# tokamak-network/Tokamak-zk-EVM

Measured on AMD Instinct MI355X. Metric: constraints/sec (prove step), higher is better.
Workload: dtype u32 limbs (255-bit Fr / 381-bit Fq modular integer arithmetic)

## Files before the change

tokamak-zk-evm_amd/csrc/msm.hip:

```cpp
#include <stdio.h>
#include <stdlib.h>

#include <algorithm>
#include <map>
#include <memory>
#include <mutex>
#include <thread>
#include <vector>

#include "common.h"
#include "ec_u.h"

#define TK_MSM_PRIMARY 1
#define TK_MSM_NS tk_msm_bls12_381
#define TK_MSM_FR_PARAMS bls12_381_fr_params
#define TK_MSM_FQ_PARAMS bls12_381_fq_params
#define TK_MSM_SCALAR_BITS 255
#define TK_MSM_ABI_FR tkmk_fr
#define TK_MSM_ABI_AFFINE tkmk_g1_affine
#define TK_MSM_ABI_PROJ tkmk_g1_projective
#define TK_MSM_ABI_JOB tkmk_msm_job
#define TK_MSM_SYM_MSM bls12_381_msm
#define TK_MSM_SYM_MULTI tkmk_msm_multi
#define TK_MSM_SYM_PRECOMPUTE bls12_381_msm_precompute_bases
#define TK_MSM_SYM_PRECOMPUTE_ACC bls12_381_msm_precompute_bases_acc
#define TK_MSM_ABI_JOB_EX tkmk_msm_job_ex
#define TK_MSM_SYM_MULTI_EX tkmk_msm_multi_ex
#define TK_MSM_SYM_CONVERT bls12_381_msm_convert_bases
#define TK_MSM_SYM_SEGMENTED tkmk_msm_segmented
#define TK_MSM_SYM_SEGMENTED_STATUS tkmk_msm_segmented_status
#include "msm_impl.inc"
```

tokamak-zk-evm_amd/csrc/msm_bn254.hip:

```cpp
#include <stdio.h>
#include <stdlib.h>

#include <algorithm>
#include <map>
#include <memory>
#include <mutex>
#include <vector>

#include "common.h"
#include "ec_u.h"

#define TK_MSM_NS tk_msm_bn254
#define TK_MSM_FR_PARAMS bn254_fr_params
#define TK_MSM_FQ_PARAMS bn254_fq_params
#define TK_MSM_SCALAR_BITS 254
#define TK_MSM_ABI_FR tkmk_bn254_fr
#define TK_MSM_ABI_AFFINE tkmk_bn254_g1_affine
#define TK_MSM_ABI_PROJ tkmk_bn254_g1_projective
#define TK_MSM_ABI_JOB tkmk_bn254_msm_job
#define TK_MSM_SYM_MSM bn254_msm
#define TK_MSM_SYM_MULTI tkmk_bn254_msm_multi
#define TK_MSM_SYM_PRECOMPUTE bn254_msm_precompute_bases
#include "msm_impl.inc"
```

tokamak-zk-evm_amd/csrc/msm_impl.inc:

```
namespace TK_MSM_NS {

using FrP = TK_MSM_FR_PARAMS;
using FqP = TK_MSM_FQ_PARAMS;
using Fr = ff<FrP>;
using Fq = ff<FqP>;
using fr_t = Fr::E;
using fq_t = Fq::E;
using G1 = ec<Fq>;
using g1_affine_t = affine_t<Fq>;
using g1_xyzz_t = xyzz_t<Fq>;
using G1U = ecu<FqP>;
using G1K = G1;
using FqK = Fq;
using g1k_xyzz = g1_xyzz_t;
using g1k_aff = g1_affine_t;
using abi_fr = TK_MSM_ABI_FR;
using abi_affine = TK_MSM_ABI_AFFINE;
using abi_proj = TK_MSM_ABI_PROJ;
using abi_job = TK_MSM_ABI_JOB;
#ifdef TK_MSM_SYM_MULTI_EX
using abi_job_ex = TK_MSM_ABI_JOB_EX;
#endif
constexpr size_t AFF_BYTES = sizeof(g1_affine_t), FR_BYTES = sizeof(fr_t);
#ifdef TK_MSM_SYM_PRECOMPUTE_ACC
// ... 46 lines not shown
__device__ __forceinline__ uint32_t view_at_expanded(const msm_view_t &v, uint32_t k, uint32_t n_src, uint32_t level_rows) {
    if (!level_rows) return view_at(v, k);
    uint32_t j = k / n_src;
    return j * level_rows + view_at(v, k - j * n_src);
}
static inline msm_view_t view_identity() { return msm_view_t{nullptr, 0, 0, 0, nullptr}; }
static inline bool view_is_identity(const msm_view_t &v) { return !v.index && !v.cols; }

__global__ __launch_bounds__(256) void k_convert_bases(const g1_affine_t *__restrict__ in, g1_affine_t *__restrict__ out,
                                                      uint64_t n, int in_montgomery, msm_view_t bv) {
    uint64_t i = (uint64_t)blockIdx.x * blockDim.x + threadIdx.x;
    if (i >= n) return;
    g1_affine_t p = tk_load(in + view_at(bv, (uint32_t)i));
    if (!G1::is_inf(p)) {
        fq_t k;
#pragma unroll
        for (int j = 0; j < Fq::N; j++) k.l[j] = in_montgomery ? FqP::KSATM[j] : FqP::KSAT[j];
        p.x = Fq::mul(Fq::canon(p.x), k);
        p.y = Fq::mul(Fq::canon(p.y), k);
    }
    tk_store(out + i, p);
}

__global__ __launch_bounds__(256) void k_digits(const fr_t *__restrict__ scalars, uint32_t *__restrict__ dig, msm_plan_t pl,
                                               int scalars_mont, msm_view_t sv) {
    uint32_t i = blockIdx.x * blockDim.x + threadIdx.x;
    if (i >= pl.n_src) return;
    fr_t s = Fr::canon(tk_load(scalars + view_at(sv, i)));
    if (scalars_mont) s = Fr::from_mont(s);
    uint32_t carry = 0;
    const uint32_t mask = (1u << pl.c) - 1u;
    const uint32_t groups = pl.n / pl.n_src;
    uint32_t j = 0, t = 0;
    for (uint32_t w = 0; w < groups * pl.W; w++) {
        if (w >= pl.W_src) {
            dig[(uint64_t)t * pl.n + (uint64_t)j * pl.n_src + i] = 0;
            if (++t == pl.W) { t = 0; j++; }
            continue;
        }
        uint32_t lo = w * pl.c, li = lo >> 5, sh = lo & 31;
        uint32_t raw = 0;
        if (li < 8) {
            raw = s.l[li] >> sh;
            if (sh + pl.c > 32 && li + 1 < 8) raw |= s.l[li + 1] << (32 - sh);
        }
        raw &= mask;
        if (lo + pl.c > pl.bits) {
            uint32_t keep = pl.bits > lo ? pl.bits - lo : 0;
            raw &= keep >= 32 ? 0xffffffffu : ((1u << keep) - 1u);
        }
        uint32_t v = raw + carry;
        uint32_t rec;
        if (v > pl.B) {
            rec = ((1u << pl.c) - v) | 0x80000000u;
            carry = 1;
        } else {
            rec = v;
            carry = 0;
        }
        dig[(uint64_t)t * pl.n + (uint64_t)j * pl.n_src + i] = rec;
        if (++t == pl.W) { t = 0; j++; }
    }
}

template <class Out>
__device__ __forceinline__ void precompute_bases_body(const g1_affine_t *__restrict__ in, Out *__restrict__ out, uint64_t n, int in_montgomery,
                                                      uint32_t factor, uint32_t step) {
    uint64_t i = (uint64_t)blockIdx.x * blockDim.x + threadIdx.x;
    if (i >= n) return;
    g1_affine_t p = tk_load(in + i);
    const bool inf = G1::is_inf(p);
    if (!inf) {
        p.x = Fq::canon(p.x);
        p.y = Fq::canon(p.y);
        if (!in_montgomery) {
            p.x = Fq::to_mont(p.x);
            p.y = Fq::to_mont(p.y);
        }
    }
    fq_t k;
#pragma unroll
    for (int l = 0; l < Fq::N; l++) k.l[l] = FqP::KSATM[l];
    g1_xyzz_t acc = G1::from_affine(p);
    for (uint32_t j = 0; j < factor; j++) {
        g1_affine_t a = p;
// ... 25 lines not shown
                                              uint32_t shift) {
    extern __shared__ uint32_t hist[];
    const uint32_t w = blockIdx.y, ch = blockIdx.x;
    for (uint32_t b = threadIdx.x; b < pl.B; b += blockDim.x) hist[b] = 0;
    __syncthreads();
    uint32_t lo = ch * pl.chunk_len, hi = lo + pl.chunk_len;
    if (hi > pl.n) hi = pl.n;
    const uint32_t *d = dig + (uint64_t)w * pl.n;
    uint32_t i = lo + threadIdx.x;
    for (; i + 3 * 1024 < hi; i += 4 * 1024) {
        uint32_t r[4];
#pragma unroll
        for (int j = 0; j < 4; j++) r[j] = d[i + 1024 * j] & 0x7fffffffu;
#pragma unroll
        for (int j = 0; j < 4; j++)
            if (r[j]) atomicAdd(&hist[(r[j] - 1) >> shift], 1u);
    }
    for (; i < hi; i += 1024) {
        uint32_t r = d[i] & 0x7fffffffu;
        if (r) atomicAdd(&hist[(r - 1) >> shift], 1u);
    }
    __syncthreads();
    uint32_t *c = counts + (uint64_t)w * pl.B * pl.chunks;
    for (uint32_t b = threadIdx.x; b < pl.B; b += blockDim.x) c[(uint64_t)b * pl.chunks + ch] = hist[b];
}

__global__ __launch_bounds__(1024) void k_scan_local(const uint32_t *__restrict__ counts, uint32_t *__restrict__ local,
                                                    uint32_t *__restrict__ gtot, msm_plan_t pl) {
    __shared__ uint32_t part[1024];
    const uint32_t w = blockIdx.y, t = threadIdx.x, b = blockIdx.x * 1024 + t;
    uint32_t sum = 0;
    if (b < pl.B) {
        const uint32_t *c = counts + ((uint64_t)w * pl.B + b) * pl.chunks;
        uint32_t k = 0;
        for (; k + 8 <= pl.chunks; k += 8) {
            uint32_t v[8];
#pragma unroll
            for (int j = 0; j < 8; j++) v[j] = c[k + j];
#pragma unroll
            for (int j = 0; j < 8; j++) sum += v[j];
        }
        for (; k < pl.chunks; k++) sum += c[k];
    }
    part[t] = sum;
    __syncthreads();
    for (uint32_t off = 1; off < 1024; off <<= 1) {
// ... 114 lines not shown
    uint32_t *s = sorted + (uint64_t)w * pl.n;
    for (uint32_t i = lo + threadIdx.x; i < hi; i += blockDim.x) {
        uint32_t rec = d[i];
        uint32_t r = rec & 0x7fffffffu;
        if (r) {
            uint32_t pos = atomicAdd(&cur[r - 1], 1u);
            s[pos] = view_at_expanded(bv, i, pl.n_src, level_rows) | (rec & 0x80000000u);
        }
    }
}

#ifndef SC_TILE
#define SC_TILE 4096
#endif
#define SC_PER (SC_TILE / 1024)
#define SC_MAXBINS 1024
#define SC_MAXFINE 512
#define SC_PARTS 4
__device__ __forceinline__ uint32_t sc_part_len(uint32_t len, uint32_t parts) {
    uint32_t per = (len + parts - 1) / parts;
    return (per + SC_TILE - 1) / SC_TILE * SC_TILE;
}

template <bool PASS_B>
__global__ __launch_bounds__(1024) void k_scatter_staged(const uint32_t *__restrict__ in0, const uint16_t *__restrict__ in1,
                                                        const uint32_t *__restrict__ seg_start, const uint32_t *__restrict__ cursors,
                                                        uint32_t *__restrict__ out0, uint16_t *__restrict__ out1, uint32_t n,
                                                        uint32_t bins, uint32_t coarse_bins, uint32_t chunk_len, uint32_t fbits,
                                                        msm_view_t bv, uint32_t n_src, uint32_t level_rows) {
    __shared__ uint32_t hist[SC_MAXBINS], start[SC_MAXBINS], cur[SC_MAXBINS], wsum[16];
    const uint32_t fmask = (1u << fbits) - 1;
    __shared__ uint32_t sv0[SC_TILE], sv1[SC_TILE];
    const uint32_t tid = threadIdx.x, parts = gridDim.x, sgm = blockIdx.y;
    uint32_t part = blockIdx.x;
    if ((parts & 7u) == 0) part = (blockIdx.x & 7u) * (parts >> 3) + (blockIdx.x >> 3);
    const uint32_t w = PASS_B ? sgm / coarse_bins : sgm;
    uint32_t lo, hi, base = 0;
    if (PASS_B) {
        const uint32_t cb = sgm - w * coarse_bins;
        const uint32_t *cs = seg_start + (uint64_t)w * (coarse_bins + 1);
        uint32_t s0 = cs[cb], s1 = cs[cb + 1];
        uint32_t per = sc_part_len(s1 - s0, parts);
        lo = s0 + part * per;
        if (lo > s1) lo = s1;
        hi = lo + per < s1 ? lo + per : s1;
        base = s0;
    } else {
        lo = part * chunk_len;
        hi = lo + chunk_len < n ? lo + chunk_len : n;
        if (lo > n) lo = n;
    }
    in0 += (uint64_t)w * n;
    if (PASS_B) in1 += (uint64_t)w * n;
    out0 += (uint64_t)w * n;
    if (!PASS_B) out1 += (uint64_t)w * n;
    if (tid < bins) cur[tid] = cursors[((uint64_t)sgm * bins + tid) * parts + part] + base;
    hist[tid] = 0;
    __syncthreads();
    for (uint32_t tlo = lo; tlo < hi; tlo += SC_TILE) {
        uint32_t v0[SC_PER], v1[SC_PER], rk[SC_PER];
        bool ok[SC_PER];
#pragma unroll
        for (int j = 0; j < SC_PER; j++) {
            uint32_t k = tlo + tid + 1024u * j;
            ok[j] = k < hi;
            v0[j] = v1[j] = rk[j] = 0;
            if (ok[j]) {
                if (PASS_B) {
                    v0[j] = in0[k];
                    v1[j] = in1[k];
                } else {
                    uint32_t rec = in0[k], r = rec & 0x7fffffffu;
                    ok[j] = r != 0;
                    v0[j] = (ok[j] ? view_at_expanded(bv, k, n_src, level_rows) : 0u) | (rec & 0x80000000u);
                    v1[j] = r - 1;
                }
            }
            if (ok[j]) rk[j] = atomicAdd(&hist[PASS_B ? (v1[j] & fmask) : (v1[j] >> fbits)], 1u);
        }
        __syncthreads();
        static_assert(SC_MAXBINS == 1024, "one bin per thread of the 1024-thread workgroup");
        const uint32_t mine = hist[tid];
        uint32_t incl = mine;
        const uint32_t lane = tid & 63u, wave = tid >> 6;
#pragma unroll
        for (uint32_t off = 1; off < 64; off <<= 1) {
            uint32_t t = __shfl_up(incl, off, 64);
            if (lane >= off) incl += t;
        }
        if (lane == 63) wsum[wave] = incl;
        __syncthreads();
        uint32_t before = 0, total = 0;
#pragma unroll
        for (uint32_t w2 = 0; w2 < 16; w2++) {
            uint32_t v = wsum[w2];
            total += v;
            if (w2 < wave) before += v;
        }
        start[tid] = before + incl - mine;
        __syncthreads();
#pragma unroll
        for (int j = 0; j < SC_PER; j++)
            if (ok[j]) {
                uint32_t b = PASS_B ? (v1[j] & fmask) : (v1[j] >> fbits);
                uint32_t pos = start[b] + rk[j];
                sv0[pos] = v0[j];
                sv1[pos] = v1[j];
            }
        __syncthreads();
#pragma unroll
        for (int j = 0; j < SC_PER; j++) {
            uint32_t k2 = tid + 1024u * j;
            if (k2 < total) {
                uint32_t a0 = sv0[k2], a1 = sv1[k2];
                uint32_t b = PASS_B ? (a1 & fmask) : (a1 >> fbits);
                uint32_t g = cur[b] + (k2 - start[b]);
                out0[g] = a0;
                if (!PASS_B) out1[g] = (uint16_t)(a1 & fmask);
            }
        }
        __syncthreads();
        cur[tid] += hist[tid];
        hist[tid] = 0;
        __syncthreads();
    }
}

__global__ __launch_bounds__(1024) void k_hist_fine(const uint16_t *__restrict__ key, const uint32_t *__restrict__ seg_start,
                                                   uint32_t *__restrict__ counts, uint32_t n, uint32_t coarse_bins, uint32_t fbits) {
    __shared__ uint32_t hist[SC_MAXFINE];
    const uint32_t fb_n = 1u << fbits;
    const uint32_t tid = threadIdx.x, part = blockIdx.x, parts = gridDim.x, sgm = blockIdx.y;
    const uint32_t w = sgm / coarse_bins, cb = sgm - w * coarse_bins;
    const uint32_t *cs = seg_start + (uint64_t)w * (coarse_bins + 1);
    uint32_t s0 = cs[cb], s1 = cs[cb + 1];
    uint32_t per = sc_part_len(s1 - s0, parts);
    uint32_t lo = s0 + part * per;
    if (lo > s1) lo = s1;
    uint32_t hi = lo + per < s1 ? lo + per : s1;
    if (tid < fb_n) hist[tid] = 0;
    __syncthreads();
    const uint16_t *k = key + (uint64_t)w * n;
    uint32_t i = lo + tid;
    for (; i + 3 * 1024 < hi; i += 4 * 1024) {
        uint32_t r[4];
#pragma unroll
        for (int j = 0; j < 4; j++) r[j] = k[i + 1024 * j];
// ... 656 lines not shown
    if (getenv("TKMK_MSM_FIXED_CHUNK")) return MSM_CHUNK;
    if (const char *e = getenv("TKMK_MSM_CHUNK_LEN")) {
        int v = atoi(e);
        if (v >= 8 && v <= 8192) return (uint32_t)v;
    }
    uint64_t target = entries / (8ull * slots);
    if (target < 48) target = 48;
    if (target > 224) target = 224;
    uint64_t r = (entries + target * slots / 2) / (target * slots);
    if (r < 1) r = 1;
    uint64_t lanes_per_window = r * slots / W;
    if (lanes_per_window < 1) lanes_per_window = 1;
    uint64_t chunk = (n + lanes_per_window - 1) / lanes_per_window;
    if (chunk < 32) chunk = 32;
    if (chunk > 256) chunk = 256;
    if (entries > (1ull << 30)) {
        uint64_t big = entries / (32ull * slots);
        if (big > 4096) big = 4096;
        if (big > chunk) chunk = big;
    }
    return (uint32_t)chunk;
}
#define MSM_MAX_C 20
static uint32_t msm_resolve_c(uint32_t c_req, uint32_t n_src) {
    uint32_t c = c_req ? c_req : choose_c(n_src);
    if (c < 2) c = 2;
    if (c > MSM_MAX_C) c = MSM_MAX_C;
    static const bool force_one_pass = getenv("TKMK_MSM_ONE_PASS") != nullptr;
    if (c > 16 && (force_one_pass || n_src < (1u << 18))) c = 16;
    return c;
}

struct msm_acc_lds_t {
    uint32_t foreground, background;
};
static const msm_acc_lds_t &msm_acc_lds() {
    static const msm_acc_lds_t claims = [] {
        const char *fg = getenv("TKMK_MSM_ACC_LDS"), *bg = getenv("TKMK_MSM_BACKGROUND_LDS");
        msm_acc_lds_t v{fg ? (uint32_t)atoi(fg) : 0u, bg ? (uint32_t)atoi(bg) : 98304u};
        const int most = (int)(v.foreground > v.background ? v.foreground : v.background);
        hipError_t e = most ? hipFuncSetAttribute((const void *)k_accumulate_chunks, hipFuncAttributeMaxDynamicSharedMemorySize, most) : hipSuccess;
#ifdef TK_MSM_SYM_PRECOMPUTE_ACC
        if (most && e == hipSuccess) e = hipFuncSetAttribute((const void *)k_accumulate_chunks_rows, hipFuncAttributeMaxDynamicSharedMemorySize, most);
#endif
        if (e != hipSuccess) v = msm_acc_lds_t{0, 0};
        return v;
    }();
    return claims;
}
static tkmk_error msm_enqueue(const fr_t *scalars, const g1_affine_t *bases_mont, uint32_t n_src, uint32_t factor, uint32_t c_req,
                              uint32_t bits, bool scalars_mont, hipStream_t s, g1_xyzz_t *wins_host, msm_plan_t *plan_out, bool background,
                              msm_view_t sv = view_identity(), msm_view_t bv = view_identity(), uint32_t level_rows = 0,
// ... 16 lines not shown
    pl.B = 1u << (pl.c - 1);
    pl.chunk = msm_choose_chunk((uint64_t)pl.W * n, pl.W, n);
    {
        static const uint32_t big_env = getenv("TKMK_MSM_BIG") ? (uint32_t)atoi(getenv("TKMK_MSM_BIG")) : 0u;
        const uint64_t avg_spans = (uint64_t)n / ((uint64_t)pl.chunk * pl.B);
        pl.big = big_env ? big_env : (avg_spans >= 4 ? 4u * MSM_BIG : MSM_BIG);
    }
    pl.win_parts = pl.W >= 8 ? MSM_WIN_PARTS : 32;
    pl.hi_bits = pl.lo_bits = 0;
    if (pl.W == 1 && pl.c >= 15) {
        pl.lo_bits = (pl.c - 1) / 2;
        pl.hi_bits = pl.c - 1 - pl.lo_bits;
    }
    static const bool no_rowcol = getenv("TKMK_MSM_SEGMENT_TAIL") != nullptr;
    if (no_rowcol) pl.hi_bits = pl.lo_bits = 0;
    uint32_t want = (512 + pl.W - 1) / pl.W;
    if (getenv("TKMK_MSM_CHUNKS")) want = (uint32_t)atoi(getenv("TKMK_MSM_CHUNKS"));
    uint32_t maxc = (n + 8191) / 8192;
    pl.chunks = want < maxc ? want : maxc;
    if (pl.chunks < 1) pl.chunks = 1;
    pl.chunk_len = (n + pl.chunks - 1) / pl.chunks;

    tk_scratch d_dig, d_sorted, d_counts, d_bstart, d_buckets, d_segs, d_wins;
    TK_TRY(d_dig.alloc((size_t)pl.W * n * 4, s));
    TK_TRY(d_sorted.alloc((size_t)pl.W * n * 4, s));
    const bool two_pass = !force_one_pass && pl.c >= 13 && n >= (1u << 18);
    if (pl.c > 16 && !two_pass) return TKMK_ERR_INVALID_ARGUMENT;
    {
        const uint32_t fb = pl.c >= 19 ? 9u : pl.c >= 17 ? 8u : 7u;
        TK_TRY(d_counts.alloc((size_t)pl.W * (two_pass ? (pl.B >> fb) : pl.B) * pl.chunks * 4, s));
    }
    TK_TRY(d_bstart.alloc((size_t)pl.W * (pl.B + 1) * 4, s));
    TK_TRY(d_buckets.alloc((size_t)pl.W * pl.B * sizeof(g1_xyzz_t), s));
    uint32_t segs = (pl.B + MSM_SEG - 1) / MSM_SEG;
    TK_TRY(d_segs.alloc((size_t)pl.W * segs * sizeof(g1_xyzz_t), s));
    TK_TRY(d_wins.alloc((size_t)pl.W * pl.win_parts * sizeof(g1_xyzz_t), s));

    tk_stat_add(TK_STAT_MSM_POINTS, n_src);
    tk_stat_add(TK_STAT_MSM_CALLS, 1);
    tk_prof prof(s);
    hipLaunchKernelGGL(k_digits, tk_div_up(n_src, 256), 256, 0, s, scalars, d_dig.as<uint32_t>(), pl, scalars_mont ? 1 : 0, sv);
    prof.mark("msm.digits");
    size_t lds = (size_t)pl.B * 4;
    static std::once_flag attr_once;
    static hipError_t attr_err = hipSuccess;
    std::call_once(attr_once, [] {
        attr_err = hipFuncSetAttribute((const void *)k_hist, hipFuncAttributeMaxDynamicSharedMemorySize, 128 * 1024);
        if (attr_err == hipSuccess)
            attr_err = hipFuncSetAttribute((const void *)k_scatter, hipFuncAttributeMaxDynamicSharedMemorySize, 128 * 1024);
    });
    TK_HIP(attr_err);
    if (!two_pass) {
        hipLaunchKernelGGL(k_hist, dim3(pl.chunks, pl.W), 1024, lds, s, (const uint32_t *)d_dig.p, d_counts.as<uint32_t>(), pl, 0u);
        prof.mark("msm.hist");
        const uint32_t groups = (pl.B + 1023) / 1024;
        tk_scratch d_local, d_gtot;
        TK_TRY(d_local.alloc((size_t)pl.W * pl.B * 4, s));
        TK_TRY(d_gtot.alloc((size_t)pl.W * groups * 4, s));
        hipLaunchKernelGGL(k_scan_local, dim3(groups, pl.W), 1024, 0, s, (const uint32_t *)d_counts.p, d_local.as<uint32_t>(),
                           d_gtot.as<uint32_t>(), pl);
        hipLaunchKernelGGL(k_scan_apply, dim3(groups, pl.W), 1024, 0, s, d_counts.as<uint32_t>(), (const uint32_t *)d_local.p,
                           (const uint32_t *)d_gtot.p, d_bstart.as<uint32_t>(), pl);
        prof.mark("msm.scan");
        hipLaunchKernelGGL(k_scatter, dim3(pl.chunks, pl.W), 1024, lds, s, (const uint32_t *)d_dig.p, (const uint32_t *)d_counts.p,
                           d_sorted.as<uint32_t>(), pl, bv, level_rows);
        prof.mark("msm.scatter");
    } else {
        const uint32_t fbits = pl.c >= 19 ? 9u : pl.c >= 17 ? 8u : 7u, FB = 1u << fbits, CB = pl.B >> fbits;
        tk_scratch d_aidx, d_akey, d_cs, d_localA, d_gtotA, d_cntB, d_fs, d_localB, d_gtotB;
        TK_TRY(d_aidx.alloc((size_t)pl.W * n * 4, s));
        TK_TRY(d_akey.alloc((size_t)pl.W * n * 2, s));
        TK_TRY(d_cs.alloc((size_t)pl.W * (CB + 1) * 4, s));
        msm_plan_t pa = pl;
        pa.B = CB;
        hipLaunchKernelGGL(k_hist, dim3(pl.chunks, pl.W), 1024, (size_t)CB * 4, s, (const uint32_t *)d_dig.p, d_counts.as<uint32_t>(), pa,
                           fbits);
        prof.mark("msm.hist");
        TK_TRY(d_localA.alloc((size_t)pl.W * CB * 4, s));
        const bool wide_scan = pl.W <= 4 && pl.chunks >= 64;
        const uint32_t groupsA = wide_scan ? (CB + SCW_BINS - 1) / SCW_BINS : 1u;
        TK_TRY(d_gtotA.alloc((size_t)pl.W * groupsA * 4, s));
        if (wide_scan) {
            hipLaunchKernelGGL(k_scan_local_wide, dim3(groupsA, pl.W), 1024, 0, s, (const uint32_t *)d_counts.p, d_localA.as<uint32_t>(),
                               d_gtotA.as<uint32_t>(), pa);
            hipLaunchKernelGGL(k_scan_apply_wide, dim3(groupsA, pl.W), 1024, 0, s, d_counts.as<uint32_t>(), (const uint32_t *)d_localA.p,
                               (const uint32_t *)d_gtotA.p, d_cs.as<uint32_t>(), pa);
        } else {
            hipLaunchKernelGGL(k_scan_local, dim3(1, pl.W), 1024, 0, s, (const uint32_t *)d_counts.p, d_localA.as<uint32_t>(),
                               d_gtotA.as<uint32_t>(), pa);
            hipLaunchKernelGGL(k_scan_apply, dim3(1, pl.W), 1024, 0, s, d_counts.as<uint32_t>(), (const uint32_t *)d_localA.p,
                               (const uint32_t *)d_gtotA.p, d_cs.as<uint32_t>(), pa);
        }
        prof.mark("msm.scan");
        hipLaunchKernelGGL(k_scatter_staged<false>, dim3(pl.chunks, pl.W), 1024, 0, s, (const uint32_t *)d_dig.p, (const uint16_t *)nullptr,
                           (const uint32_t *)nullptr, (const uint32_t *)d_counts.p, d_aidx.as<uint32_t>(), d_akey.as<uint16_t>(), n, CB, CB,
                           pl.chunk_len, fbits, bv, pl.n_src, level_rows);
        const uint32_t segs_b = pl.W * CB;
        TK_TRY(d_cntB.alloc((size_t)segs_b * FB * SC_PARTS * 4, s));
        TK_TRY(d_fs.alloc((size_t)segs_b * (FB + 1) * 4, s));
        TK_TRY(d_localB.alloc((size_t)segs_b * FB * 4, s));
        TK_TRY(d_gtotB.alloc((size_t)segs_b * 4, s));
        hipLaunchKernelGGL(k_hist_fine, dim3(SC_PARTS, segs_b), 1024, 0, s, (const uint16_t *)d_akey.p, (const uint32_t *)d_cs.p,
                           d_cntB.as<uint32_t>(), n, CB, fbits);
        msm_plan_t pb = pl;
        pb.B = FB;
        pb.chunks = SC_PARTS;
        hipLaunchKernelGGL(k_scan_local, dim3(1, segs_b), 1024, 0, s, (const uint32_t *)d_cntB.p, d_localB.as<uint32_t>(),
                           d_gtotB.as<uint32_t>(), pb);
        hipLaunchKernelGGL(k_scan_apply, dim3(1, segs_b), 1024, 0, s, d_cntB.as<uint32_t>(), (const uint32_t *)d_localB.p,
                           (const uint32_t *)d_gtotB.p, d_fs.as<uint32_t>(), pb);
        hipLaunchKernelGGL(k_bstart_assemble, tk_div_up((size_t)pl.W * (pl.B + 1), 256), 256, 0, s, (const uint32_t *)d_cs.p,
                           (const uint32_t *)d_fs.p, d_bstart.as<uint32_t>(), pl.W, pl.B, CB, fbits);
        hipLaunchKernelGGL(k_scatter_staged<true>, dim3(SC_PARTS, segs_b), 1024, 0, s, (const uint32_t *)d_aidx.p, (const uint16_t *)d_akey.p,
                           (const uint32_t *)d_cs.p, (const uint32_t *)d_cntB.p, d_sorted.as<uint32_t>(), (uint16_t *)nullptr, n, FB, CB,
                           0u, fbits, view_identity(), 0u, 0u);
        prof.mark("msm.scatter");
    }
    if (unsigned long long *cell = tk_stat_device_entries())
        hipLaunchKernelGGL(k_count_entries, 1, 1, 0, s, (const uint32_t *)d_bstart.p, pl.W, pl.B, cell);
    const uint32_t cpw = (n + pl.chunk - 1) / pl.chunk;
    const uint32_t big_cap = pl.W * pl.B;
    tk_scratch d_fh, d_ft, d_big, d_giant, d_gpart;
    TK_TRY(d_fh.alloc((size_t)pl.W * cpw * sizeof(g1_xyzz_t), s));
    TK_TRY(d_ft.alloc((size_t)pl.W * cpw * sizeof(g1_xyzz_t), s));
    TK_TRY(d_big.alloc((size_t)(big_cap + 1) * 4, s));
    TK_TRY(d_giant.alloc((size_t)(MSM_GIANT_CAP + 1) * 4, s));
    TK_TRY(d_gpart.alloc((size_t)MSM_GIANT_CAP * MSM_GIANT_PARTS * sizeof(g1_xyzz_t), s));
    TK_HIP(hipMemsetAsync(d_buckets.p, 0, (size_t)pl.W * pl.B * sizeof(g1_xyzz_t), s));
    TK_HIP(hipMemsetAsync(d_big.p, 0, 4, s));
    TK_HIP(hipMemsetAsync(d_giant.p, 0, 4, s));
    const msm_acc_lds_t &acc_lds = msm_acc_lds();
    const uint32_t lds_claim = (background && acc_lds.background) ? acc_lds.background : acc_lds.foreground;
    prof.mark("msm.prepare");
#ifdef TK_MSM_SYM_PRECOMPUTE_ACC
    if (acc_rows)
        hipLaunchKernelGGL(k_accumulate_chunks_rows, tk_div_up((size_t)pl.W * cpw, 256), 256, lds_claim, s, acc_rows, (const uint32_t *)d_sorted.p,
                           (const uint32_t *)d_bstart.p, d_buckets.as<g1_xyzz_t>(), d_fh.as<g1_xyzz_t>(), d_ft.as<g1_xyzz_t>(), pl, cpw);
    else
// ... 14 lines not shown
    prof.mark("msm.combine");
    size_t wins_count = (size_t)pl.W * pl.win_parts;
    if (pl.lo_bits) {
        const uint32_t HI = 1u << pl.hi_bits, LO = 1u << pl.lo_bits;
        g1_xyzz_t *rows = d_segs.as<g1_xyzz_t>(), *cols = rows + HI;
        hipLaunchKernelGGL(k_reduce_rows_cols, HI / 4 + LO / 2, 256, 0, s, (const g1_xyzz_t *)d_buckets.p, rows, cols, HI, LO);
        prof.mark("msm.reduce_segments");
        wins_count = 1 + pl.hi_bits + pl.lo_bits;
        hipLaunchKernelGGL(k_reduce_bits, (unsigned)wins_count, 256, 0, s, (const g1_xyzz_t *)rows, (const g1_xyzz_t *)cols, HI, LO, pl.hi_bits,
                           d_wins.as<g1_xyzz_t>());
        prof.mark("msm.reduce_windows");
    } else {
        hipLaunchKernelGGL(k_reduce_segments, tk_div_up((size_t)pl.W * segs, 128), 128, 0, s, (const g1_xyzz_t *)d_buckets.p,
                           d_segs.as<g1_xyzz_t>(), pl, segs);
        prof.mark("msm.reduce_segments");
        hipLaunchKernelGGL(k_reduce_windows, dim3(pl.W, pl.win_parts), 256, 0, s, (const g1_xyzz_t *)d_segs.p, d_wins.as<g1_xyzz_t>(), segs, pl.win_parts);
        prof.mark("msm.reduce_windows");
    }
    TK_HIP(hipGetLastError());
    if (getenv("TKMK_MSM_DEBUG"))
        fprintf(stderr, "[msm debug] ptrs dig=%p sorted=%p counts=%p bstart=%p buckets=%p (+%zu) segs=%p (+%zu) wins=%p\n", d_dig.p,
                d_sorted.p, d_counts.p, d_bstart.p, d_buckets.p, (size_t)pl.W * pl.B * sizeof(g1_xyzz_t), d_segs.p,
                (size_t)pl.W * segs * sizeof(g1_xyzz_t), d_wins.p);
    if (getenv("TKMK_MSM_DEBUG") && factor == 1 && view_is_identity(sv) && view_is_identity(bv) && !level_rows && !acc_rows) TK_TRY(msm_debug_check(pl, scalars, bases_mont, d_dig.as<uint32_t>(), d_sorted.as<uint32_t>(),
                                                          d_bstart.as<uint32_t>(), d_buckets.as<g1_xyzz_t>(), s));
    TK_HIP(hipMemcpyAsync(wins_host, d_wins.p, wins_count * sizeof(g1_xyzz_t), hipMemcpyDeviceToHost, s));
    prof.finish();
    *plan_out = pl;
    return TKMK_SUCCESS;
}

static g1_xyzz_t msm_horner(const msm_plan_t &pl, const g1_xyzz_t *wins) {
    if (pl.lo_bits) {
        g1_xyzz_t hi = G1::inf(), lo = G1::inf();
        for (int k = (int)pl.hi_bits - 1; k >= 0; k--) hi = G1::add(G1::dbl(hi), G1U::raw_to_sat(wins[1 + k]));
        for (int k = (int)pl.lo_bits - 1; k >= 0; k--) lo = G1::add(G1::dbl(lo), G1U::raw_to_sat(wins[1 + pl.hi_bits + k]));
        for (uint32_t k = 0; k < pl.lo_bits; k++) hi = G1::dbl(hi);
        return G1::add(G1::add(G1U::raw_to_sat(wins[0]), hi), lo);
    }
    g1_xyzz_t acc = G1::inf();
    for (int w = (int)pl.W - 1; w >= 0; w--) {
        for (uint32_t k = 0; k < pl.c; k++) acc = G1::dbl(acc);
        for (uint32_t part = 0; part < pl.win_parts; part++) acc = G1::add(acc, G1U::raw_to_sat(wins[w * pl.win_parts + part]));
    }
    return acc;
}

// ... 331 lines not shown
    if (!cfg->are_scalars_on_device || !cfg->are_points_on_device) return TKMK_ERR_INVALID_ARGUMENT;
    if (n_jobs == 0) return TKMK_SUCCESS;
    if (!jobs || !results) return TKMK_ERR_INVALID_POINTER;
    TK_TRY(tk_require_device());
    const uint32_t bits = cfg->bitsize ? (uint32_t)cfg->bitsize : (uint32_t)TK_MSM_SCALAR_BITS;
    hipStream_t s = tk_stream(cfg->stream_handle);
    tk_frame frame(s);
    for (int j = 0; j < n_jobs; j++) {
        const abi_job_ex &jb = jobs[j];
        if (jb.msm_size < 0) return TKMK_ERR_INVALID_ARGUMENT;
        if (jb.msm_size > 0 && (!jb.scalars || !jb.bases)) return TKMK_ERR_INVALID_POINTER;
        if ((jb.scalar_cols && jb.scalar_stride < jb.scalar_cols) || (jb.base_cols && jb.base_stride < jb.base_cols)) return TKMK_ERR_INVALID_ARGUMENT;
        if (jb.msm_size > 0 && jb.base_cols && !jb.base_index && jb.base_table_len) {
            uint64_t last = (uint64_t)((uint32_t)jb.msm_size - 1) / jb.base_cols * jb.base_stride + ((uint32_t)jb.msm_size - 1) % jb.base_cols;
            if (last >= jb.base_table_len) return TKMK_ERR_INVALID_ARGUMENT;
        }
        if (jb.base_table_len >= (1ull << 31)) return TKMK_ERR_INVALID_ARGUMENT;
        if (jb.msm_size > 0 && jb.base_index && !jb.base_table_len) return TKMK_ERR_INVALID_ARGUMENT;
        if ((jb.table_c != 0) != (jb.table_factor != 0)) return TKMK_ERR_INVALID_ARGUMENT;
        if (acc_ready && jb.table_c != 0 && jb.table_factor < 2) return TKMK_ERR_INVALID_ARGUMENT;
        if (jb.table_factor > 1) {
            if (bases_form != TKMK_BASES_CONVERTED || !jb.base_table_len || jb.table_c < 2 || jb.table_c > MSM_MAX_C) return TKMK_ERR_INVALID_ARGUMENT;
            if (jb.base_table_len * jb.table_factor >= (1ull << 31)) return TKMK_ERR_INVALID_ARGUMENT;
            if (jb.table_c > 16 && (uint64_t)jb.msm_size * jb.table_factor < (1ull << 18)) return TKMK_ERR_INVALID_ARGUMENT;
            if (acc_ready) {
                if (((uintptr_t)jb.bases & (ACC_ROW_BYTES - 1)) != 0 || jb.msm_size == 1) return TKMK_ERR_INVALID_ARGUMENT;
            }
        }
    }
    tk_scratch d_flag;
    TK_TRY(d_flag.alloc(4, s));
    TK_HIP(hipMemsetAsync(d_flag.p, 0, 4, s));
    std::vector<abi_proj> host_res(n_jobs);
    std::vector<msm_pipe_job> pj;
    std::vector<int> pj_index;
    for (int j = 0; j < n_jobs; j++) {
        const abi_job_ex &jb = jobs[j];
        if (jb.msm_size < 2) {
            TK_TRY(msm_ex_tiny(jb, cfg, bases_form, &host_res[j]));
            continue;
        }
        msm_view_t sv{nullptr, jb.scalar_cols, jb.scalar_stride, 0, nullptr};
        msm_view_t bv{jb.base_index, jb.base_index ? 0u : jb.base_cols, jb.base_index ? 0u : jb.base_stride,
                      jb.base_index ? (uint32_t)jb.base_table_len : 0u, d_flag.as<uint32_t>()};
        msm_pipe_job pjob{(const fr_t *)jb.scalars, (const g1_affine_t *)jb.bases, (uint32_t)jb.msm_size, bases_form != TKMK_BASES_CONVERTED,
                          bases_form == TKMK_BASES_MONTGOMERY, 1u, sv, bv};
        if (jb.table_factor > 1) {
// ... 251 lines not shown
```

Measured before the change: 20.21 million.

## Fuse signed-digit recoding into MSM histogram and scatter passes, skipping digit array

```diff
diff --git a/tokamak-zk-evm_amd/csrc/msm.hip b/tokamak-zk-evm_amd/csrc/msm.hip
--- a/tokamak-zk-evm_amd/csrc/msm.hip
+++ b/tokamak-zk-evm_amd/csrc/msm.hip
@@ -10,6 +10,7 @@
 
 #include "common.h"
 #include "ec_u.h"
+#include "msm_recode.h"
 
 #define TK_MSM_PRIMARY 1
 #define TK_MSM_NS tk_msm_bls12_381
diff --git a/tokamak-zk-evm_amd/csrc/msm_bn254.hip b/tokamak-zk-evm_amd/csrc/msm_bn254.hip
--- a/tokamak-zk-evm_amd/csrc/msm_bn254.hip
+++ b/tokamak-zk-evm_amd/csrc/msm_bn254.hip
@@ -9,6 +9,7 @@
 
 #include "common.h"
 #include "ec_u.h"
+#include "msm_recode.h"
 
 #define TK_MSM_NS tk_msm_bn254
 #define TK_MSM_FR_PARAMS bn254_fr_params
diff --git a/tokamak-zk-evm_amd/csrc/msm_impl.inc b/tokamak-zk-evm_amd/csrc/msm_impl.inc
--- a/tokamak-zk-evm_amd/csrc/msm_impl.inc
+++ b/tokamak-zk-evm_amd/csrc/msm_impl.inc
@@ -92,45 +92,18 @@
     tk_store(out + i, p);
 }
 
+__device__ __forceinline__ msm_recode_t msm_recode_of(const msm_plan_t &pl, int scalars_mont) {
+    return msm_recode_t{pl.c, pl.W_src, pl.bits, (pl.n / pl.n_src) * pl.W, scalars_mont};
+}
 __global__ __launch_bounds__(256) void k_digits(const fr_t *__restrict__ scalars, uint32_t *__restrict__ dig, msm_plan_t pl,
                                                int scalars_mont, msm_view_t sv) {
     uint32_t i = blockIdx.x * blockDim.x + threadIdx.x;
     if (i >= pl.n_src) return;
-    fr_t s = Fr::canon(tk_load(scalars + view_at(sv, i)));
-    if (scalars_mont) s = Fr::from_mont(s);
-    uint32_t carry = 0;
-    const uint32_t mask = (1u << pl.c) - 1u;
-    const uint32_t groups = pl.n / pl.n_src;
     uint32_t j = 0, t = 0;
-    for (uint32_t w = 0; w < groups * pl.W; w++) {
-        if (w >= pl.W_src) {
-            dig[(uint64_t)t * pl.n + (uint64_t)j * pl.n_src + i] = 0;
-            if (++t == pl.W) { t = 0; j++; }
-            continue;
-        }
-        uint32_t lo = w * pl.c, li = lo >> 5, sh = lo & 31;
-        uint32_t raw = 0;
-        if (li < 8) {
-            raw = s.l[li] >> sh;
-            if (sh + pl.c > 32 && li + 1 < 8) raw |= s.l[li + 1] << (32 - sh);
-        }
-        raw &= mask;
-        if (lo + pl.c > pl.bits) {
-            uint32_t keep = pl.bits > lo ? pl.bits - lo : 0;
-            raw &= keep >= 32 ? 0xffffffffu : ((1u << keep) - 1u);
-        }
-        uint32_t v = raw + carry;
-        uint32_t rec;
-        if (v > pl.B) {
-            rec = ((1u << pl.c) - v) | 0x80000000u;
-            carry = 1;
-        } else {
-            rec = v;
-            carry = 0;
-        }
+    msm_recode<Fr>(tk_load(scalars + view_at(sv, i)), msm_recode_of(pl, scalars_mont), [&](uint32_t, uint32_t rec) {
         dig[(uint64_t)t * pl.n + (uint64_t)j * pl.n_src + i] = rec;
         if (++t == pl.W) { t = 0; j++; }
-    }
+    });
 }
 
 template <class Out>
@@ -202,6 +175,31 @@
     }
     __syncthreads();
     uint32_t *c = counts + (uint64_t)w * pl.B * pl.chunks;
+    for (uint32_t b = threadIdx.x; b < pl.B; b += blockDim.x) c[(uint64_t)b * pl.chunks + ch] = hist[b];
+}
+
+__global__ __launch_bounds__(1024) void k_hist_points(const fr_t *__restrict__ scalars, uint32_t *__restrict__ counts, msm_plan_t pl,
+                                                     uint32_t shift, uint32_t pchunk, int scalars_mont, msm_view_t sv) {
+    extern __shared__ uint32_t hist[];
+    const uint32_t ch = blockIdx.x;
+    for (uint32_t b = threadIdx.x; b < pl.B; b += blockDim.x) hist[b] = 0;
+    __syncthreads();
+    uint32_t lo = ch * pchunk, hi = lo + pchunk;
+    if (hi > pl.n_src) hi = pl.n_src;
+    const msm_recode_t rc = msm_recode_of(pl, scalars_mont);
+    auto count = [&](uint32_t, uint32_t rec) {
+        const uint32_t r = rec & 0x7fffffffu;
+        if (r) atomicAdd(&hist[(r - 1) >> shift], 1u);
+    };
+    uint32_t i = lo + threadIdx.x;
+    for (; i + 1024 < hi; i += 2 * 1024) {
+        const fr_t a = tk_load(scalars + view_at(sv, i)), b = tk_load(scalars + view_at(sv, i + 1024));
+        msm_recode<Fr>(a, rc, count);
+        msm_recode<Fr>(b, rc, count);
+    }
+    for (; i < hi; i += 1024) msm_recode<Fr>(tk_load(scalars + view_at(sv, i)), rc, count);
+    __syncthreads();
+    uint32_t *c = counts;
     for (uint32_t b = threadIdx.x; b < pl.B; b += blockDim.x) c[(uint64_t)b * pl.chunks + ch] = hist[b];
 }
 
@@ -362,16 +360,30 @@
     return (per + SC_TILE - 1) / SC_TILE * SC_TILE;
 }
 
-template <bool PASS_B>
-__global__ __launch_bounds__(1024) void k_scatter_staged(const uint32_t *__restrict__ in0, const uint16_t *__restrict__ in1,
+enum { SC_A_DIG = 0, SC_A_POINTS = 1, SC_B = 2 };
+struct sc_points_t {
+    const fr_t *scalars;
+    msm_view_t sv;
+    msm_recode_t rc;
+};
+__device__ __forceinline__ uint32_t sc_tile_points(uint32_t levels) {
+    uint32_t tp = SC_TILE / (levels + 1);
+    return tp < 1024u ? tp : 1024u;
+}
+
+template <int MODE>
+__global__ __launch_bounds__(1024, 8) void k_scatter_staged(const uint32_t *__restrict__ in0, const uint16_t *__restrict__ in1,
                                                         const uint32_t *__restrict__ seg_start, const uint32_t *__restrict__ cursors,
                                                         uint32_t *__restrict__ out0, uint16_t *__restrict__ out1, uint32_t n,
                                                         uint32_t bins, uint32_t coarse_bins, uint32_t chunk_len, uint32_t fbits,
-                                                        msm_view_t bv, uint32_t n_src, uint32_t level_rows) {
-    __shared__ uint32_t hist[SC_MAXBINS], start[SC_MAXBINS], cur[SC_MAXBINS], wsum[16];
+                                                        msm_view_t bv, uint32_t n_src, uint32_t level_rows, sc_points_t pt) {
+    constexpr bool PASS_B = MODE == SC_B, POINTS = MODE == SC_A_POINTS;
+    static_assert(SC_MAXBINS == 1024, "one bin per thread of the 1024-thread workgroup");
+    __shared__ uint32_t hist[SC_MAXBINS], startw[SC_MAXBINS], gofs[SC_MAXBINS], wsum[16];
+    __shared__ uint32_t sv0[SC_TILE], sv1[SC_TILE];
+    __shared__ uint32_t stage[POINTS ? 2 : 1][POINTS ? SC_TILE : 1];
     const uint32_t fmask = (1u << fbits) - 1;
-    __shared__ uint32_t sv0[SC_TILE], sv1[SC_TILE];
-    const uint32_t tid = threadIdx.x, parts = gridDim.x, sgm = blockIdx.y;
+    const uint32_t tid = threadIdx.x, lane = tid & 63u, wave = tid >> 6, parts = gridDim.x, sgm = blockIdx.y;
     uint32_t part = blockIdx.x;
     if ((parts & 7u) == 0) part = (blockIdx.x & 7u) * (parts >> 3) + (blockIdx.x >> 3);
     const uint32_t w = PASS_B ? sgm / coarse_bins : sgm;
@@ -386,67 +398,123 @@
         hi = lo + per < s1 ? lo + per : s1;
         base = s0;
     } else {
+        const uint32_t items = POINTS ? n_src : n;
         lo = part * chunk_len;
-        hi = lo + chunk_len < n ? lo + chunk_len : n;
-        if (lo > n) lo = n;
-    }
-    in0 += (uint64_t)w * n;
+        hi = lo + chunk_len < items ? lo + chunk_len : items;
+        if (lo > items) lo = items;
+    }
+    if (!POINTS) in0 += (uint64_t)w * n;
     if (PASS_B) in1 += (uint64_t)w * n;
     out0 += (uint64_t)w * n;
     if (!PASS_B) out1 += (uint64_t)w * n;
-    if (tid < bins) cur[tid] = cursors[((uint64_t)sgm * bins + tid) * parts + part] + base;
+    uint32_t cur = tid < bins ? cursors[((uint64_t)sgm * bins + tid) * parts + part] + base : 0u;
     hist[tid] = 0;
+
+    const uint32_t levels = POINTS ? pt.rc.nwin : 1u, TP = POINTS ? sc_tile_points(levels) : 0u;
+    const uint32_t step = POINTS ? TP : (uint32_t)SC_TILE;
+    const uint32_t tp_inv = POINTS ? 0xffffffffu / TP + 1u : 0u;
+    uint32_t n0[SC_PER], n1[SC_PER];
+    fr_t nxt;
+#pragma unroll
+    for (int j = 0; j < SC_PER; j++) n0[j] = n1[j] = 0;
+#pragma unroll
+    for (int l = 0; l < 8; l++) nxt.l[l] = 0;
+    auto load_entries = [&](uint32_t t0) {
+#pragma unroll
+        for (int j = 0; j < SC_PER; j++) {
+            uint32_t k = t0 + tid + 1024u * j;
+            if (k >= hi) k = hi - 1;
+            n0[j] = in0[k];
+            if (PASS_B) n1[j] = in1[k];
+        }
+    };
+    auto load_points = [&](uint32_t t0) {
+        uint32_t i = t0 + (tid < TP ? tid : 0u);
+        if (i >= hi) i = hi - 1;
+        nxt = tk_load(pt.scalars + view_at(pt.sv, i));
+    };
+    const uint32_t lstride = level_rows ? level_rows : n_src;
+    auto stage_points = [&](uint32_t t0, uint32_t buf) {
+        if (tid < TP && t0 + tid < hi) {
+            msm_recode<Fr>(nxt, pt.rc, [&](uint32_t lv, uint32_t rec) { stage[buf][lv * TP + tid] = rec; });
+            stage[buf][levels * TP + tid] = view_at(bv, t0 + tid);
+        }
+    };
+    if (POINTS) {
+        for (uint32_t q = 0; q < 2; q++)
+            if (lo + q * step < hi) {
+                load_points(lo + q * step);
+                stage_points(lo + q * step, q);
+            }
+        if (lo + 2 * step < hi) load_points(lo + 2 * step);
+    } else if (lo < hi)
+        load_entries(lo);
     __syncthreads();
-    for (uint32_t tlo = lo; tlo < hi; tlo += SC_TILE) {
+    uint32_t tb = 0;
+    for (uint32_t tlo = lo; tlo < hi; tlo += step, tb ^= 1u) {
         uint32_t v0[SC_PER], v1[SC_PER], rk[SC_PER];
         bool ok[SC_PER];
 #pragma unroll
         for (int j = 0; j < SC_PER; j++) {
-            uint32_t k = tlo + tid + 1024u * j;
-            ok[j] = k < hi;
-            v0[j] = v1[j] = rk[j] = 0;
-            if (ok[j]) {
-                if (PASS_B) {
-                    v0[j] = in0[k];
-                    v1[j] = in1[k];
+            rk[j] = 0;
+            if (PASS_B) {
+                ok[j] = tlo + tid + 1024u * j < hi;
+                v0[j] = n0[j];
+                v1[j] = n1[j];
+            } else {
+                uint32_t rec, row = 0;
+                if (POINTS) {
+                    uint32_t e = tid + 1024u * j;
+                    asm volatile("" : "+v"(e));
+                    const uint32_t ej = __umulhi(e, tp_inv), ep = e - ej * TP;
+                    ok[j] = ej < levels && tlo + ep < hi;
+                    rec = ok[j] ? stage[tb][e] : 0u;
+                    if (ok[j]) row = ej * lstride + stage[tb][levels * TP + ep];
+                    ok[j] = ok[j] && (rec & 0x7fffffffu) != 0;
                 } else {
-                    uint32_t rec = in0[k], r = rec & 0x7fffffffu;
-                    ok[j] = r != 0;
-                    v0[j] = (ok[j] ? view_at_expanded(bv, k, n_src, level_rows) : 0u) | (rec & 0x80000000u);
-                    v1[j] = r - 1;
+                    const uint32_t k = tlo + tid + 1024u * j;
+                    rec = n0[j];
+                    ok[j] = k < hi && (rec & 0x7fffffffu) != 0;
+                    if (ok[j]) row = view_at_expanded(bv, k, n_src, level_rows);
                 }
+                v0[j] = (ok[j] ? row : 0u) | (rec & 0x80000000u);
+                v1[j] = (rec & 0x7fffffffu) - 1;
             }
             if (ok[j]) rk[j] = atomicAdd(&hist[PASS_B ? (v1[j] & fmask) : (v1[j] >> fbits)], 1u);
         }
         __syncthreads();
-        static_assert(SC_MAXBINS == 1024, "one bin per thread of the 1024-thread workgroup");
         const uint32_t mine = hist[tid];
+        hist[tid] = 0;
         uint32_t incl = mine;
-        const uint32_t lane = tid & 63u, wave = tid >> 6;
 #pragma unroll
         for (uint32_t off = 1; off < 64; off <<= 1) {
             uint32_t t = __shfl_up(incl, off, 64);
             if (lane >= off) incl += t;
         }
+        startw[tid] = incl - mine;
         if (lane == 63) wsum[wave] = incl;
         __syncthreads();
-        uint32_t before = 0, total = 0;
-#pragma unroll
-        for (uint32_t w2 = 0; w2 < 16; w2++) {
-            uint32_t v = wsum[w2];
-            total += v;
-            if (w2 < wave) before += v;
-        }
-        start[tid] = before + incl - mine;
-        __syncthreads();
-#pragma unroll
-        for (int j = 0; j < SC_PER; j++)
+        const uint32_t wtot = lane < 16 ? wsum[lane & 15u] : 0u;
+        uint32_t wincl = wtot;
+#pragma unroll
+        for (uint32_t off = 1; off < 16; off <<= 1) {
+            uint32_t t = __shfl_up(wincl, off, 64);
+            if (lane >= off) wincl += t;
+        }
+        const uint32_t wpre = wincl - wtot, total = __shfl(wincl, 15, 64);
+        gofs[tid] = cur - (__shfl(wpre, (int)wave, 64) + incl - mine);
+        cur += mine;
+#pragma unroll
+        for (int j = 0; j < SC_PER; j++) {
+            const uint32_t b = ok[j] ? (PASS_B ? (v1[j] & fmask) : (v1[j] >> fbits)) : 0u;
+            const uint32_t wp = __shfl(wpre, (int)(b >> 6), 64);
             if (ok[j]) {
-                uint32_t b = PASS_B ? (v1[j] & fmask) : (v1[j] >> fbits);
-                uint32_t pos = start[b] + rk[j];
+                uint32_t pos = startw[b] + wp + rk[j];
                 sv0[pos] = v0[j];
                 sv1[pos] = v1[j];
             }
+        }
+        if (!POINTS && tlo + step < hi) load_entries(tlo + step);
         __syncthreads();
 #pragma unroll
         for (int j = 0; j < SC_PER; j++) {
@@ -454,15 +522,15 @@
             if (k2 < total) {
                 uint32_t a0 = sv0[k2], a1 = sv1[k2];
                 uint32_t b = PASS_B ? (a1 & fmask) : (a1 >> fbits);
-                uint32_t g = cur[b] + (k2 - start[b]);
+                uint32_t g = gofs[b] + k2;
                 out0[g] = a0;
                 if (!PASS_B) out1[g] = (uint16_t)(a1 & fmask);
             }
         }
-        __syncthreads();
-        cur[tid] += hist[tid];
-        hist[tid] = 0;
-        __syncthreads();
+        if (POINTS && tlo + 2 * step < hi) {
+            stage_points(tlo + 2 * step, tb);
+            if (tlo + 3 * step < hi) load_points(tlo + 3 * step);
+        }
     }
 }
 
@@ -1165,12 +1233,16 @@
     return (uint32_t)chunk;
 }
 #define MSM_MAX_C 20
+static uint32_t msm_two_pass_min() {
+    const char *e = getenv("TKMK_MSM_TWO_PASS_MIN");
+    return e ? (uint32_t)atoi(e) : (1u << 18);
+}
 static uint32_t msm_resolve_c(uint32_t c_req, uint32_t n_src) {
     uint32_t c = c_req ? c_req : choose_c(n_src);
     if (c < 2) c = 2;
     if (c > MSM_MAX_C) c = MSM_MAX_C;
     static const bool force_one_pass = getenv("TKMK_MSM_ONE_PASS") != nullptr;
-    if (c > 16 && (force_one_pass || n_src < (1u << 18))) c = 16;
+    if (c > 16 && (force_one_pass || n_src < msm_two_pass_min())) c = 16;
     return c;
 }
 
@@ -1233,9 +1305,11 @@
     pl.chunk_len = (n + pl.chunks - 1) / pl.chunks;
 
     tk_scratch d_dig, d_sorted, d_counts, d_bstart, d_buckets, d_segs, d_wins;
-    TK_TRY(d_dig.alloc((size_t)pl.W * n * 4, s));
+    const bool two_pass = !force_one_pass && pl.c >= 13 && n >= msm_two_pass_min();
+    static const bool keep_dig = getenv("TKMK_MSM_DIGIT_ARRAY") != nullptr;
+    const bool from_points = two_pass && pl.W == 1 && !keep_dig;
+    if (!from_points) TK_TRY(d_dig.alloc((size_t)pl.W * n * 4, s));
     TK_TRY(d_sorted.alloc((size_t)pl.W * n * 4, s));
-    const bool two_pass = !force_one_pass && pl.c >= 13 && n >= (1u << 18);
     if (pl.c > 16 && !two_pass) return TKMK_ERR_INVALID_ARGUMENT;
     {
         const uint32_t fb = pl.c >= 19 ? 9u : pl.c >= 17 ? 8u : 7u;
@@ -1250,8 +1324,10 @@
     tk_stat_add(TK_STAT_MSM_POINTS, n_src);
     tk_stat_add(TK_STAT_MSM_CALLS, 1);
     tk_prof prof(s);
-    hipLaunchKernelGGL(k_digits, tk_div_up(n_src, 256), 256, 0, s, scalars, d_dig.as<uint32_t>(), pl, scalars_mont ? 1 : 0, sv);
-    prof.mark("msm.digits");
+    if (!from_points) {
+        hipLaunchKernelGGL(k_digits, tk_div_up(n_src, 256), 256, 0, s, scalars, d_dig.as<uint32_t>(), pl, scalars_mont ? 1 : 0, sv);
+        prof.mark("msm.digits");
+    }
     size_t lds = (size_t)pl.B * 4;
     static std::once_flag attr_once;
     static hipError_t attr_err = hipSuccess;
@@ -1284,8 +1360,13 @@
         TK_TRY(d_cs.alloc((size_t)pl.W * (CB + 1) * 4, s));
         msm_plan_t pa = pl;
         pa.B = CB;
-        hipLaunchKernelGGL(k_hist, dim3(pl.chunks, pl.W), 1024, (size_t)CB * 4, s, (const uint32_t *)d_dig.p, d_counts.as<uint32_t>(), pa,
-                           fbits);
+        const uint32_t pchunk = (n_src + pl.chunks - 1) / pl.chunks;
+        if (from_points)
+            hipLaunchKernelGGL(k_hist_points, dim3(pl.chunks), 1024, (size_t)CB * 4, s, scalars, d_counts.as<uint32_t>(), pa, fbits, pchunk,
+                               scalars_mont ? 1 : 0, sv);
+        else
+            hipLaunchKernelGGL(k_hist, dim3(pl.chunks, pl.W), 1024, (size_t)CB * 4, s, (const uint32_t *)d_dig.p, d_counts.as<uint32_t>(), pa,
+                               fbits);
         prof.mark("msm.hist");
         TK_TRY(d_localA.alloc((size_t)pl.W * CB * 4, s));
         const bool wide_scan = pl.W <= 4 && pl.chunks >= 64;
@@ -1303,9 +1384,16 @@
                                (const uint32_t *)d_gtotA.p, d_cs.as<uint32_t>(), pa);
         }
         prof.mark("msm.scan");
-        hipLaunchKernelGGL(k_scatter_staged<false>, dim3(pl.chunks, pl.W), 1024, 0, s, (const uint32_t *)d_dig.p, (const uint16_t *)nullptr,
-                           (const uint32_t *)nullptr, (const uint32_t *)d_counts.p, d_aidx.as<uint32_t>(), d_akey.as<uint16_t>(), n, CB, CB,
-                           pl.chunk_len, fbits, bv, pl.n_src, level_rows);
+        const sc_points_t no_points{nullptr, view_identity(), msm_recode_t{0, 0, 0, 0, 0}};
+        if (from_points)
+            hipLaunchKernelGGL(k_scatter_staged<SC_A_POINTS>, dim3(pl.chunks, 1), 1024, 0, s, (const uint32_t *)nullptr, (const uint16_t *)nullptr,
+                               (const uint32_t *)nullptr, (const uint32_t *)d_counts.p, d_aidx.as<uint32_t>(), d_akey.as<uint16_t>(), n, CB, CB,
+                               pchunk, fbits, bv, pl.n_src, level_rows,
+                               sc_points_t{scalars, sv, msm_recode_t{pl.c, pl.W_src, pl.bits, n / n_src, scalars_mont ? 1 : 0}});
+        else
+            hipLaunchKernelGGL(k_scatter_staged<SC_A_DIG>, dim3(pl.chunks, pl.W), 1024, 0, s, (const uint32_t *)d_dig.p, (const uint16_t *)nullptr,
+                               (const uint32_t *)nullptr, (const uint32_t *)d_counts.p, d_aidx.as<uint32_t>(), d_akey.as<uint16_t>(), n, CB, CB,
+                               pl.chunk_len, fbits, bv, pl.n_src, level_rows, no_points);
         const uint32_t segs_b = pl.W * CB;
         TK_TRY(d_cntB.alloc((size_t)segs_b * FB * SC_PARTS * 4, s));
         TK_TRY(d_fs.alloc((size_t)segs_b * (FB + 1) * 4, s));
@@ -1322,9 +1410,9 @@
                            (const uint32_t *)d_gtotB.p, d_fs.as<uint32_t>(), pb);
         hipLaunchKernelGGL(k_bstart_assemble, tk_div_up((size_t)pl.W * (pl.B + 1), 256), 256, 0, s, (const uint32_t *)d_cs.p,
                            (const uint32_t *)d_fs.p, d_bstart.as<uint32_t>(), pl.W, pl.B, CB, fbits);
-        hipLaunchKernelGGL(k_scatter_staged<true>, dim3(SC_PARTS, segs_b), 1024, 0, s, (const uint32_t *)d_aidx.p, (const uint16_t *)d_akey.p,
+        hipLaunchKernelGGL(k_scatter_staged<SC_B>, dim3(SC_PARTS, segs_b), 1024, 0, s, (const uint32_t *)d_aidx.p, (const uint16_t *)d_akey.p,
                            (const uint32_t *)d_cs.p, (const uint32_t *)d_cntB.p, d_sorted.as<uint32_t>(), (uint16_t *)nullptr, n, FB, CB,
-                           0u, fbits, view_identity(), 0u, 0u);
+                           0u, fbits, view_identity(), 0u, 0u, no_points);
         prof.mark("msm.scatter");
     }
     if (unsigned long long *cell = tk_stat_device_entries())
@@ -1385,7 +1473,7 @@
         fprintf(stderr, "[msm debug] ptrs dig=%p sorted=%p counts=%p bstart=%p buckets=%p (+%zu) segs=%p (+%zu) wins=%p\n", d_dig.p,
                 d_sorted.p, d_counts.p, d_bstart.p, d_buckets.p, (size_t)pl.W * pl.B * sizeof(g1_xyzz_t), d_segs.p,
                 (size_t)pl.W * segs * sizeof(g1_xyzz_t), d_wins.p);
-    if (getenv("TKMK_MSM_DEBUG") && factor == 1 && view_is_identity(sv) && view_is_identity(bv) && !level_rows && !acc_rows) TK_TRY(msm_debug_check(pl, scalars, bases_mont, d_dig.as<uint32_t>(), d_sorted.as<uint32_t>(),
+    if (getenv("TKMK_MSM_DEBUG") && factor == 1 && view_is_identity(sv) && view_is_identity(bv) && !level_rows && !acc_rows && d_dig.p) TK_TRY(msm_debug_check(pl, scalars, bases_mont, d_dig.as<uint32_t>(), d_sorted.as<uint32_t>(),
                                                           d_bstart.as<uint32_t>(), d_buckets.as<g1_xyzz_t>(), s));
     TK_HIP(hipMemcpyAsync(wins_host, d_wins.p, wins_count * sizeof(g1_xyzz_t), hipMemcpyDeviceToHost, s));
     prof.finish();
@@ -1763,7 +1851,7 @@
         if (jb.table_factor > 1) {
             if (bases_form != TKMK_BASES_CONVERTED || !jb.base_table_len || jb.table_c < 2 || jb.table_c > MSM_MAX_C) return TKMK_ERR_INVALID_ARGUMENT;
             if (jb.base_table_len * jb.table_factor >= (1ull << 31)) return TKMK_ERR_INVALID_ARGUMENT;
-            if (jb.table_c > 16 && (uint64_t)jb.msm_size * jb.table_factor < (1ull << 18)) return TKMK_ERR_INVALID_ARGUMENT;
+            if (jb.table_c > 16 && (uint64_t)jb.msm_size * jb.table_factor < msm_two_pass_min()) return TKMK_ERR_INVALID_ARGUMENT;
             if (acc_ready) {
                 if (((uintptr_t)jb.bases & (ACC_ROW_BYTES - 1)) != 0 || jb.msm_size == 1) return TKMK_ERR_INVALID_ARGUMENT;
             }
diff --git a/tokamak-zk-evm_amd/csrc/msm_recode.h b/tokamak-zk-evm_amd/csrc/msm_recode.h
--- /dev/null
+++ b/tokamak-zk-evm_amd/csrc/msm_recode.h
@@ -0,0 +1,44 @@
+#pragma once
+#include <stdint.h>
+
+#include "ff.h"
+
+struct msm_recode_t {
+    uint32_t c;
+    uint32_t W_src;
+    uint32_t bits;
+    uint32_t nwin;
+    int from_mont;
+};
+
+template <class F, class Emit>
+FF_HD void msm_recode(const typename F::E &raw, const msm_recode_t &rc, Emit &&emit) {
+    static_assert(F::N == 8, "8 scalar limbs");
+    typename F::E s = F::canon(raw);
+    if (rc.from_mont) s = F::from_mont(s);
+#pragma unroll
+    for (int l = 0; l < 8; l++) {
+        const uint32_t lo = 32u * l;
+        if (rc.bits <= lo) s.l[l] = 0;
+        else if (rc.bits < lo + 32u) s.l[l] &= (1u << (rc.bits - lo)) - 1u;
+    }
+    const uint32_t mask = (1u << rc.c) - 1u, B = 1u << (rc.c - 1);
+    uint32_t carry = 0;
+    for (uint32_t w = 0; w < rc.nwin; w++) {
+        if (w >= rc.W_src) {
+            emit(w, 0u);
+            continue;
+        }
+        const uint32_t v = (s.l[0] & mask) + carry;
+        uint32_t rec = v;
+        carry = 0;
+        if (v > B) {
+            rec = ((1u << rc.c) - v) | 0x80000000u;
+            carry = 1;
+        }
+        emit(w, rec);
+#pragma unroll
+        for (int l = 0; l < 7; l++) s.l[l] = (s.l[l] >> rc.c) | (s.l[l + 1] << (32u - rc.c));
+        s.l[7] >>= rc.c;
+    }
+}
```

Result: slower. 19.81 million (-2.0%).
